# quanwei0/RAGEN

Hardware: AMD Instinct MI355X
Metric: env-steps/sec (whole node), Sokoban 6x6, 8192 envs x 5 turns (higher is better)
Workload: dtype u8

## Files before the change

ragen_amd/csrc/board_step.hpp:

```cpp
#pragma once
#include <stdint.h>
#if defined(__HIPCC__)
#include <hip/hip_runtime.h>
#endif

#include "ragen_amd.h"

#if defined(__HIP_DEVICE_COMPILE__)
#define RMI_BS_FN __device__ __forceinline__
#elif defined(__HIPCC__)
#define RMI_BS_FN __host__ __device__ __forceinline__
#else
#define RMI_BS_FN inline
#endif

namespace rmi {
namespace bs {

RMI_BS_FN uint32_t ubfe(uint32_t x, uint32_t off, uint32_t w) {
#if defined(__HIP_DEVICE_COMPILE__)
  return __builtin_amdgcn_ubfe(x, off, w);
#else
  off &= 31u;
  w &= 31u;
  return w ? (x >> off) & ((1u << w) - 1u) : 0u;
#endif
}
RMI_BS_FN uint32_t smask(uint32_t x, uint32_t off, uint32_t w) {
#if defined(__HIP_DEVICE_COMPILE__)
  return (uint32_t)__builtin_amdgcn_sbfe((int32_t)x, off, w);
#else
  off &= 31u;
  w &= 31u;
  return w ? (uint32_t)((int32_t)(x << (32u - off - w)) >> (32u - w)) : 0u;
#endif
}
template <class T>
RMI_BS_FN void opaque(T& x) {
#if defined(__HIP_DEVICE_COMPILE__)
  asm("" : "+v"(x));
#else
  (void)x;
#endif
}
RMI_BS_FN int32_t sbyte(uint32_t x, uint32_t off) {
#if defined(__HIP_DEVICE_COMPILE__)
  return __builtin_amdgcn_sbfe((int32_t)x, off, 8u);
#else
  return (int32_t)(int8_t)(uint8_t)(x >> off);
#endif
}
RMI_BS_FN uint32_t pick_bytes(uint32_t table, uint32_t sel) {
#if defined(__HIP_DEVICE_COMPILE__)
  return __builtin_amdgcn_perm(0u, table, sel);
#else
  uint32_t r = 0;
  for (int i = 0; i < 4; ++i) r |= ((table >> (8 * ((sel >> (8 * i)) & 3u))) & 0xFFu) << (8 * i);
  return r;
#endif
}
RMI_BS_FN int popc32(uint32_t x) { return __builtin_popcount(x); }
RMI_BS_FN int popc64(uint64_t x) { return __builtin_popcountll(x); }

template <class M>
struct Word;
template <>
struct Word<uint32_t> {
  static RMI_BS_FN uint32_t mask(uint32_t x, int j) { return smask(x, (uint32_t)j, 1u); }
  static RMI_BS_FN uint32_t at(int j) { return 1u << (j & 31); }
  static RMI_BS_FN uint32_t widen(uint32_t m) { return m; }
  static RMI_BS_FN int popc(uint32_t x) { return popc32(x); }
};
template <>
struct Word<uint64_t> {
  static RMI_BS_FN uint32_t mask(uint64_t x, int j) { return 0u - ((uint32_t)(x >> (j & 63)) & 1u); }
  static RMI_BS_FN uint64_t at(int j) { return 1ull << (j & 63); }
  static RMI_BS_FN uint64_t widen(uint32_t m) { return (uint64_t)(int64_t)(int32_t)m; }
  static RMI_BS_FN int popc(uint64_t x) { return popc64(x); }
};

RMI_BS_FN uint32_t valid_bytes(uint32_t x, uint32_t in_range) {
  return ((((x & 0x7F7F7F7Fu) + 0x7F7F7F7Fu) | x) & 0x80808080u) & in_range;
}

struct Slots4 {
  uint32_t V, P, D, S;
};
RMI_BS_FN Slots4 slots4(uint32_t x, uint32_t valid, uint32_t below, uint32_t left_b, uint32_t m_b, uint32_t dir_table) {
  Slots4 s;
  const uint32_t pc = (valid >> 7) * 0x01010101u + below;
  s.V = ((left_b | 0x80808080u) - pc) & valid;
  s.P = s.V & ~((x & 0x7F7F7F7Fu) + 0x7B7B7B7Bu);
  s.D = s.V & ~((pc ^ m_b) + 0x7F7F7F7Fu);
  s.S = pick_bytes(dir_table, x & 0x03030303u);
  return s;
}

struct BoardTurn {
  double acc;
  uint32_t info, taken, stop, succ, moved;
  int nes, bot;
};

template <class M, int K>
RMI_BS_FN BoardTurn board_turn_k(M wall, M target, M& box, int& jp, int W, uint64_t acts, int n_act, int left,
                                 int nes, int bot, int num_boxes, int max_steps) {
  const M box0 = box;
  const int jp0 = jp;
  const uint32_t dir_table = 0x01u | ((uint32_t)(-W) & 0xFFu) << 8 | ((uint32_t)W & 0xFFu) << 16 | 0xFF000000u;
  const uint64_t range = n_act >= 8 ? ~0ull : (1ull << (8 * n_act)) - 1;
  const uint32_t l8 = left <= 0 ? 0u : (left >= 8 ? 8u : (uint32_t)left);
  const int m = max_steps - nes;
  const uint32_t m8 = (m >= 1 && m <= 8) ? (uint32_t)m : 0x7Fu;
  const uint32_t left_b = l8 * 0x01010101u, m_b = m8 * 0x01010101u;
  const uint32_t xl = (uint32_t)acts, xh = (uint32_t)(acts >> 32);
  const uint32_t vl = valid_bytes(xl, (uint32_t)range);
  Slots4 q[2];
  q[0] = slots4(xl, vl, 0u, left_b, m_b, dir_table);
  if (K > 4) q[1] = slots4(xh, valid_bytes(xh, (uint32_t)(range >> 32)), (uint32_t)popc32(vl) * 0x01010101u, left_b, m_b, dir_table);
  uint32_t alive = 1u, taken = 0u, last_moved = 0u, z = 1u;
  int open_bot = num_boxes - bot;
  double acc = 0.0;
#pragma unroll
  for (int k = 0; k < K; ++k) {
    const Slots4& v = q[k >> 2];
    const uint32_t hb = 8u * (uint32_t)(k & 3) + 7u;
    const int s = sbyte(v.S, 8u * (uint32_t)(k & 3));
    const uint32_t go = smask(v.V, hb, alive), go_push = smask(v.P, hb, alive), go_done = smask(v.D, hb, alive);
    const int jn = jp + s, jb = jn + s;
    const M occ = wall | box;
    const uint32_t n_box = Word<M>::mask(box, jn), n_occ = Word<M>::mask(occ, jn), b_occ = Word<M>::mask(occ, jb);
    const uint32_t is_push = go_push & n_box & ~b_occ;
    const uint32_t moved = go & (is_push | ~n_occ);
    box ^= (Word<M>::at(jn) | Word<M>::at(jb)) & Word<M>::widen(is_push);
    jp = (int)((moved & (uint32_t)jn) | (~moved & (uint32_t)jp));
    const int n_open = Word<M>::popc(target & ~box);
    int sg = n_open - open_bot;
    sg = sg > 1 ? 1 : (sg < -1 ? -1 : sg);
    z = n_open < 1 ? (uint32_t)n_open : 1u;
    uint32_t fin = 1u - z;
    opaque(sg);
    opaque(fin);
    double rw = -0.1 - (double)sg;
    rw = __builtin_fma(10.0, (double)fin, rw);
    acc = __builtin_fma(-(double)(int32_t)go, rw, acc);
    open_bot = (int)((go & (uint32_t)n_open) | (~go & (uint32_t)open_bot));
    taken -= go;
    last_moved = (go & moved) | (~go & last_moved);
    alive &= ~(go_done | (go & fin));
  }
  BoardTurn t;
  t.acc = acc;
  t.taken = taken;
  t.stop = alive ^ 1u;
  t.succ = taken ? (z ^ 1u) : 0u;
  t.info = taken ? (RMI_INFO_PRESENT | RMI_INFO_VALID | (last_moved & 2u) | (t.succ << 3)) : 0u;
  t.moved = (box != box0) | (jp != jp0);
  t.nes = nes + (int)taken;
  t.bot = num_boxes - open_bot;
  return t;
}

}
}
```

ragen_amd/csrc/sokoban.hip:

```cpp
#include "common.hpp"
#include "board_step.hpp"
#include "parse_core.hpp"

#include <type_traits>

namespace rmi {
namespace {

constexpr int kWave = 64;
constexpr int kMaxCells = 64;

__device__ __forceinline__ uint32_t zero_bytes(uint32_t y) {
  return ~(((y & 0x7F7F7F7Fu) + 0x7F7F7F7Fu) | y) & 0x80808080u;
}
__device__ __forceinline__ uint32_t eq_bytes(uint32_t x, uint32_t v) { return zero_bytes(x ^ (v * 0x01010101u)); }

struct SokobanLdsEnv {
  uint8_t* st;
  const uint8_t* fx;
  int H, W, r, c;
  int num_env_steps, boxes_on_target, num_boxes, max_steps, n_open;
  uint8_t err;

  __device__ __forceinline__ int wrap(int row, int col, bool& ok) const {
    ok = row >= -H && row < H && col >= -W && col < W;
    const int rr = row < 0 ? row + H : row, cc = col < 0 ? col + W : col;
    return ok ? rr * W + cc : 0;
  }
  __device__ __forceinline__ static int open_of(int v, int f) { return (v == 2) | ((v == 5) & (f == 2)); }

  __device__ __forceinline__ bool step(int a, double& reward, bool& done, bool& eff, bool& success) {
    if (a < 1 || a > 8) return false;
    const int d = (a - 1) & 3;
    const int dr = d == 0 ? -1 : (d == 1 ? 1 : 0);
    const int dc = d == 2 ? -1 : (d == 3 ? 1 : 0);
    const int nr = r + dr, nc = c + dc, br = nr + dr, bc = nc + dc;
    bool ok_n, ok_b, ok_o;
    const int ni = wrap(nr, nc, ok_n), bi = wrap(br, bc, ok_b), oi = wrap(r, c, ok_o);
    const int vn = st[ni], vb = st[bi], vo = st[oi];
    const int fn = fx[ni], fb = fx[bi], fo = fx[oi];
    const bool push_act = a <= 4;
    const bool high = br >= H || bc >= W;
    const bool is_push = push_act && !high && (vn == 3 || vn == 4) && (vb == 1 || vb == 2);
    const bool try_move = !push_act || (!high && !is_push);
    const bool moved = is_push || (try_move && (vn == 1 || vn == 2));
    if ((push_act && !high && (!ok_n || !ok_b)) || (try_move && !ok_n) || (moved && !ok_o)) {
      err |= RMI_ERR_INDEX;
      return false;
    }
    num_env_steps += 1;
    const int vbn = fb == 2 ? 3 : 4;
    if (moved) {
      n_open += open_of(5, fn) - open_of(vn, fn) + open_of(fo, fo) - open_of(vo, fo);
      st[ni] = 5;
      st[oi] = (uint8_t)fo;
      r = nr;
      c = nc;
    }
    if (is_push) {
      n_open += open_of(vbn, fb) - open_of(vb, fb);
      st[bi] = (uint8_t)vbn;
    }
    const int cur = num_boxes - n_open;
    double rw = -0.1;
    rw += cur > boxes_on_target ? 1.0 : (cur < boxes_on_target ? -1.0 : 0.0);
    const bool all_on = n_open == 0;
    rw += all_on ? 10.0 : 0.0;
    boxes_on_target = cur;
    reward = rw;
    done = all_on || (max_steps == num_env_steps);
    success = boxes_on_target == num_boxes;
    eff = moved;
    return true;
  }
};

struct ExecList {
  uint64_t run;
  int cnt;
};
__device__ __forceinline__ ExecList exec_list(uint64_t acts, int n_act, int left) {
  ExecList x;
  x.run = 0;
  x.cnt = 0;
#pragma unroll
  for (int k = 0; k < kMaxK; ++k) {
    const uint32_t a = (uint32_t)(acts >> (8 * k)) & 0xFFu;
    const bool take = k < n_act && a != 0 && x.cnt < left;
    x.run |= take ? ((uint64_t)a << (8 * x.cnt)) : 0ull;
    x.cnt += take;
  }
  return x;
}

__device__ __forceinline__ void finish_turn(const TurnOut& o, bool turn_done, bool succ_last, int32_t& num_actions,
                                            uint8_t& flags, int32_t& n_turns, int max_actions) {
  num_actions += o.exec;
  n_turns += 1;
  if (turn_done) {
    flags |= RMI_FLAG_TERMINATED | RMI_FLAG_DONE;
    flags = succ_last ? (uint8_t)(flags & ~RMI_FLAG_TRUNCATED) : (uint8_t)(flags | RMI_FLAG_TRUNCATED);
  } else if (num_actions >= max_actions) {
    flags |= RMI_FLAG_TERMINATED | RMI_FLAG_TRUNCATED | RMI_FLAG_DONE;
  }
}

__device__ __forceinline__ double step_reward(int n_open, int num_boxes, int& boxes_on_target, bool& all_on) {
  const int cur = num_boxes - n_open;
  double rw = -0.1;
  rw += cur > boxes_on_target ? 1.0 : (cur < boxes_on_target ? -1.0 : 0.0);
  all_on = n_open == 0;
  rw += all_on ? 10.0 : 0.0;
  boxes_on_target = cur;
  return rw;
}


__device__ __forceinline__ uint32_t nonzero_bytes(uint32_t y) {
  return (((y & 0x7F7F7F7Fu) + 0x7F7F7F7Fu) | y) & 0x80808080u;
}
__device__ __forceinline__ uint32_t gt8_bytes(uint32_t y) {
  return (y | ((y & 0x7F7F7F7Fu) + 0x77777777u)) & 0x80808080u;
}
__device__ __forceinline__ uint32_t nib(uint32_t x) { return (x * 0x01020408u) >> 24; }
__device__ __forceinline__ uint32_t nib2(uint32_t x0, uint32_t x1) {
  return ((x0 | (x1 << 4)) * 0x00204081u) >> 21 & 0xFFu;
}
__device__ __forceinline__ uint32_t byte_mask(uint32_t x) { return (0x80808080u - x) ^ 0x80808080u; }

template <int LPE>
__device__ __forceinline__ uint32_t env_or(uint32_t x) {
  if (LPE >= 2) x |= (uint32_t)__builtin_amdgcn_mov_dpp((int)x, 0xB1, 0xF, 0xF, false);
  if (LPE >= 4) x |= (uint32_t)__builtin_amdgcn_mov_dpp((int)x, 0x4E, 0xF, 0xF, false);
  if (LPE >= 8) x |= (uint32_t)__builtin_amdgcn_mov_dpp((int)x, 0x141, 0xF, 0xF, false);
  if (LPE >= 16) x |= (uint32_t)__builtin_amdgcn_mov_dpp((int)x, 0x140, 0xF, 0xF, false);
  static_assert(LPE <= 16, "an env's lanes lie in one DPP row");
  return x;
}
template <int LPE>
__device__ __forceinline__ uint64_t env_or64(uint64_t x) {
  return ((uint64_t)env_or<LPE>((uint32_t)(x >> 32)) << 32) | env_or<LPE>((uint32_t)x);
}

template <int NWL, int LPE>
__device__ __forceinline__ bool decode_rows(const uint32_t (&xs)[NWL], const uint32_t (&xf)[NWL], int sub,
                                            int row_words, int p, uint64_t& wall, uint64_t& target, uint64_t& box) {
  constexpr uint32_t L = 0x01010101u;
  const int pw = p >> 2;
  const uint32_t pmask = 0xFFu << (8 * (p & 3)), p5 = 5u << (8 * (p & 3));
  uint32_t bad = 0;
  uint64_t wl = 0, tl = 0, bl = 0;
  uint32_t fw[NWL], ft[NWL], bx[NWL];
#pragma unroll
  for (int i = 0; i < NWL; ++i) {
// ... 564 lines not shown
        if (w < row_words) {
          ls[w] = xs[i];
          lf[w] = xf[i];
        }
      }
    }
    wave_sync();
    if (act && sub == 0) {
      int n_open = 0;
      for (int w = 0; w < row_words; ++w)
        n_open += __popc(eq_bytes(ls[w], 2u) | (eq_bytes(ls[w], 5u) & eq_bytes(lf[w], 2u)));
      SokobanLdsEnv e;
      e.st = reinterpret_cast<uint8_t*>(ls);
      e.fx = reinterpret_cast<const uint8_t*>(lf);
      e.H = H;
      e.W = W;
      e.r = r;
      e.c = c;
      e.num_env_steps = nes;
      e.boxes_on_target = bot;
      e.num_boxes = env.num_boxes;
      e.max_steps = env.max_steps;
      e.n_open = n_open;
      e.err = 0;
      const ExecList x = exec_list(acts, n_act, left);
      o = lds_turn(e, x, err, turn_done, succ_last);
      err |= e.err;
      r = e.r;
      c = e.c;
      nes = e.num_env_steps;
      bot = e.boxes_on_target;
      row_changed = o.stepped_any_state;
    }
    wave_sync();
    row_changed = env_or<LPE>(row_changed) != 0;
    if (act && row_changed) {
#pragma unroll
      for (int i = 0; i < NWL; ++i) {
        const int w = sub + LPE * i;
        if (w < row_words) xs[i] = ls[w];
      }
    }
  }
  RMI_STAMP(3);

  if (kFirst && live && !act && sub == 0) {
    elem<Ix>(env.player, 2 * b)[0] = (int8_t)r;
    elem<Ix>(env.player, 2 * b)[1] = (int8_t)c;
    *elem<Ix>(env.num_env_steps, b) = 0;
    *elem<Ix>(env.boxes_on_target, b) = 0;
    *elem<Ix>(ep.num_actions, b) = 0;
    *elem<Ix>(ep.flags, b) = 0;
    *elem<Ix>(ep.n_turns, b) = 0;
    *elem<Ix>(ep.penalty, b) = 0.0;
  }
  if (kFirst && live && sub == 0)
    for (int t = 0; t < ep.T; ++t)
      if (t != in.turn || !act) {
        *elem<Ix>(ep.turn_reward + (int64_t)t * B, b) = 0.0;
        *elem<Ix>(ep.turn_info + (int64_t)t * B, b) = 0;
        *elem<Ix>(ep.turn_exec + (int64_t)t * B, b) = 0;
      }
  if (act) {
    if (sub == 0) {
      finish_turn(o, turn_done, succ_last, num_actions, flags, n_turns, in.max_actions_per_traj);
      *elem<Ix>(ep.num_actions, b) = num_actions;
      *elem<Ix>(ep.flags, b) = flags;
      *elem<Ix>(ep.n_turns, b) = n_turns;
      *elem<Ix>(ep.penalty, b) = penalty;
      const int64_t tb = (int64_t)in.turn * B;
      *elem<Ix>(ep.turn_reward + tb, b) = o.acc;
      *elem<Ix>(ep.turn_info + tb, b) = o.info;
      *elem<Ix>(ep.turn_exec + tb, b) = o.exec;
      if (kFirst || o.stepped_any_state) {
        elem<Ix>(env.player, 2 * b)[0] = (int8_t)r;
        elem<Ix>(env.player, 2 * b)[1] = (int8_t)c;
        *elem<Ix>(env.num_env_steps, b) = nes;
        *elem<Ix>(env.boxes_on_target, b) = bot;
      }
      if (err_out && err) *elem<Ix>(err_out, b) |= err;
    }
    if (row_changed) store_row<NWL, LPE, HW != 0>(elem<Ix>(env.room_state, b * hw), xs, sub, row_words);
  }
  if (bmode != RMI_BOARDS_NONE && live) {
    const bool stepped_fast = fast && act;
    const bool write = bmode == RMI_BOARDS_BUILD || act || kFirst;
    const uint32_t tag = (stepped_fast || !act) ? (from_cache || room_ok ? 1u : 0u) : 0u;
    if (write) {
      const uint32_t cell = (uint32_t)(jp + W) & 0xFFu;
      *elem<Ix>(reinterpret_cast<Dw4*>(env.boards), b) = Dw4{(uint32_t)wall, (uint32_t)target, (uint32_t)box,
                                                   cell | (tag << 8) | ((uint32_t)nes & 0xFFu) << 16 |
                                                       ((uint32_t)bot & 0xFFu) << 24};
    }
  }
  RMI_STAMP(4);
  at_end(xs, xf, wall, target, box, (fast && act) ? jp : INT32_MIN);
  if (kFin) {
    if (act) rec.set(in.turn, o.acc, o.info);
    finalize_envs<LPE, Ix>(ep, fin, rec, b, live && sub == 0, flags, n_turns, num_actions, penalty, act ? in.turn : -1,
                       o.acc, o.info);
  }
}

template <int HW, class M, int LPE, bool kFin, bool kFirst = false, bool kLate = false, bool kObs = false,
          class Ix = int64_t>
__global__ __launch_bounds__(kWave * kSokWpb * (kObs ? kObsFan : 1)) void sokoban_step_turn_kernel(rmi_sokoban_t env, rmi_episode_t ep, rmi_turn_t in,
                                                                  int hw_rt, uint32_t w_magic, uint64_t border,
                                                                  uint8_t* __restrict__ err_out, rmi_finalize_t fin,
                                                                  const uint8_t* __restrict__ init_state = nullptr,
                                                                  const int8_t* __restrict__ init_player = nullptr,
                                                                  ObsOut obs = ObsOut{}) {
  static_assert(!kObs || (HW == 36 && LPE == 1 && !kLate), "the fused render: 36-cell rooms, one lane per env");
  constexpr int NW = HW ? HW / 4 : kMaxWords;
  constexpr int kEnvs = kWave / LPE;
  __shared__ uint32_t lds_state[kSokWpb * kEnvs * NW];
  __shared__ uint32_t lds_fixed[kSokWpb * kEnvs * NW];
  using ObsL = ObsLds<kObs ? HW : 36, M>;
  __shared__ typename std::conditional<kObs, ObsL, char>::type lds_obs;
  const int B = ep.B;
  const int lane = threadIdx.x & (kWave - 1), wave = threadIdx.x / kWave;
  const int sub = lane % LPE, slot = lane / LPE;
  const bool turn_wave = !kObs || wave < kSokWpb;
  const int64_t b = turn_wave ? ((int64_t)blockIdx.x * kSokWpb + wave) * kEnvs + slot : (int64_t)B;
  const int row_words = (HW ? HW : hw_rt) >> 2;
  auto at_end = [&](const auto& xs, const auto& xf, M wall, M target, M box, int jp) {
        if constexpr (kObs) {
          const int H = env.H, W = env.W;
          if (turn_wave) {
            const int e = wave * kWave + lane;
#pragma unroll
            for (int i = 0; i < NW; ++i) {
              lds_obs.xs[e][i] = xs[i];
              lds_obs.xf[e][i] = xf[i];
            }
            lds_obs.wall[e] = wall;
            lds_obs.target[e] = target;
            lds_obs.box[e] = box;
            lds_obs.jp[e] = jp;
          }
          if (threadIdx.x < 18) lds_obs.gb[threadIdx.x] = threadIdx.x < 16 ? obs.gb[threadIdx.x] : (threadIdx.x == 16 ? '?' : '\n');
          __syncthreads();
#ifndef RMI_OBS_SKIP_RENDER
          render_group<HW, M>(obs, lds_obs, B, H, W);
#endif
        }
      };
  constexpr bool kBoards = HW == 36 && LPE == 1 && !kLate && !kObs && sizeof(M) == 4;
  static_assert(sizeof(Ix) == 8 || kBoards, "32-bit env offsets: the SK layout only (launched below kOff32MaxB envs)");
  turn_env<HW, M, LPE, kFin, kFirst, kLate, kBoards, Ix>(env, ep, in, hw_rt, w_magic, border, err_out, fin, init_state,
                                                         init_player, b, sub, lds_state + (wave * kEnvs + slot) * row_words,
                                                         lds_fixed + (wave * kEnvs + slot) * row_words, at_end);
}

__global__ __launch_bounds__(kBlock) void sokoban_reset_kernel(rmi_sokoban_t env, rmi_episode_t ep, int hw,
                                                               const uint8_t* __restrict__ init_state,
                                                               const int8_t* __restrict__ init_player) {
  const int64_t i = (int64_t)blockIdx.x * kBlock + threadIdx.x;
  const int64_t B = ep.B;
  const int64_t nwords = (B * hw) >> 2;
  if (i < nwords) reinterpret_cast<uint32_t*>(env.room_state)[i] = reinterpret_cast<const uint32_t*>(init_state)[i];
  if (i < B) {
    env.player[2 * i] = init_player[2 * i];
    env.player[2 * i + 1] = init_player[2 * i + 1];
    env.num_env_steps[i] = 0;
    env.boxes_on_target[i] = 0;
    ep.num_actions[i] = 0;
    ep.flags[i] = 0;
    ep.n_turns[i] = 0;
    ep.penalty[i] = 0.0;
    for (int t = 0; t < ep.T; ++t) {
      ep.turn_reward[t * B + i] = 0.0;
      ep.turn_info[t * B + i] = 0;
      ep.turn_exec[t * B + i] = 0;
    }
  }
}

__global__ __launch_bounds__(kBlock) void sokoban_load_rooms_kernel(rmi_sokoban_t env, rmi_episode_t ep, int hw,
                                                                    const uint8_t* __restrict__ rooms, int n_rooms,
                                                                    const int32_t* __restrict__ room_of,
                                                                    uint8_t* __restrict__ init_state,
                                                                    int8_t* __restrict__ init_player,
                                                                    uint8_t* __restrict__ err) {
  const int64_t t = (int64_t)blockIdx.x * kBlock + threadIdx.x;
  const int64_t B = ep.B;
  const int64_t pitch = 2 * hw + 2;
  if (t < B * hw) {
    const int64_t i = t / hw;
    const int k = (int)(t - i * hw);
    const int r = room_of ? room_of[i] : (int)i;
    const bool bad = r < 0 || r >= n_rooms;
    const uint8_t f = bad ? 0 : rooms[(int64_t)r * pitch + k], v = bad ? 0 : rooms[(int64_t)r * pitch + hw + k];
    const_cast<uint8_t*>(env.room_fixed)[t] = f;
    env.room_state[t] = v;
    init_state[t] = v;
  }
  if (t < B) {
    const int64_t i = t;
    const int r = room_of ? room_of[i] : (int)i;
    const bool bad = r < 0 || r >= n_rooms;
    if (err) err[i] = bad ? RMI_ERR_INDEX : 0;
    const uint8_t* src = rooms + (int64_t)(bad ? 0 : r) * pitch + 2 * hw;
    const int8_t p0 = bad ? 0 : (int8_t)src[0], p1 = bad ? 0 : (int8_t)src[1];
    init_player[2 * i] = p0;
    init_player[2 * i + 1] = p1;
    env.player[2 * i] = p0;
    env.player[2 * i + 1] = p1;
    env.num_env_steps[i] = 0;
    env.boxes_on_target[i] = 0;
    ep.num_actions[i] = 0;
    ep.flags[i] = 0;
    ep.n_turns[i] = 0;
    ep.penalty[i] = 0.0;
    for (int u = 0; u < ep.T; ++u) {
      ep.turn_reward[u * B + i] = 0.0;
      ep.turn_info[u * B + i] = 0;
      ep.turn_exec[u * B + i] = 0;
    }
  }
}


constexpr int kTokEnvs = 16;
#ifdef RMI_TOK_STAMPS
__device__ unsigned long long* g_tok_stamps;
#define TST_DECL unsigned long long tst_[8] = {0}; tst_[0] = __builtin_amdgcn_s_memrealtime(); tst_[1] = __builtin_amdgcn_s_memtime()
#define TST(i) (tst_[i] = __builtin_amdgcn_s_memtime())
#define TST_FLUSH(w)                                                                              \
  do {                                                                                            \
    tst_[7] = __builtin_amdgcn_s_memrealtime();                                                   \
    if ((threadIdx.x & 63) == 0 && g_tok_stamps)                                                  \
      for (int s_ = 0; s_ < 8; ++s_) g_tok_stamps[((int64_t)blockIdx.x * kTokEnvs + (w)) * 8 + s_] = tst_[s_]; \
  } while (0)
#else
#define TST_DECL do {} while (0)
#define TST(i) do {} while (0)
#define TST_FLUSH(w) do {} while (0)
#endif
constexpr int kTokRowWords = 48;
struct TokRec {
  uint32_t xs[9], xf[9];
  uint32_t wall, target, box;
  int jp;
};
__host__ __device__ constexpr size_t tok_static_lds() {
  return 2 * kTokEnvs * 9 * 4 + kTokEnvs * sizeof(TokRec) + kTokEnvs * kTokRowWords * 4 + 18 * 4;
}

template <bool kFin, bool kFirst>
__global__ __launch_bounds__(kWave* kTokEnvs) __attribute__((amdgpu_waves_per_eu(8))) void sokoban_token_turn_kernel(
    DetokArgs d, ParseArgs a, rmi_sokoban_t env, rmi_episode_t ep, rmi_turn_t in, uint32_t w_magic, uint64_t border,
    uint8_t* __restrict__ err_out, rmi_finalize_t fin, const uint8_t* __restrict__ init_state,
    const int8_t* __restrict__ init_player, ObsOut obs, const uint8_t* __restrict__ has_t, uint8_t* __restrict__ has) {
  extern __shared__ uint64_t lds_q[];
  __shared__ uint32_t lds_state[kTokEnvs * 9], lds_fixed[kTokEnvs * 9];
  __shared__ TokRec rec[kTokEnvs];
  __shared__ uint32_t blk[kTokEnvs][kTokRowWords];
  __shared__ uint32_t gb[18];
  __shared__ struct {
    uint8_t* out;
    int32_t* len;
    uint64_t glen;
    int stride, H, W, B;
  } rp;
  const int wv = __builtin_amdgcn_readfirstlane(threadIdx.x >> 6), lane = threadIdx.x & 63;
  const int64_t b0 = (int64_t)blockIdx.x * kTokEnvs, b = b0 + wv;
  TST_DECL;
  if (threadIdx.x < 18) gb[threadIdx.x] = threadIdx.x < 16 ? obs.gb[threadIdx.x] : (threadIdx.x == 16 ? '?' : '\n');
  if (threadIdx.x == 64) {
    rp.out = obs.out;
    rp.len = obs.len;
    rp.glen = obs.glen;
    rp.stride = obs.stride;
    rp.H = env.H;
    rp.W = env.W;
    rp.B = ep.B;
  }

  if (b < a.B) {
    uint8_t* lds = reinterpret_cast<uint8_t*>(lds_q) + wv * parse_lds(a.stride);
    const int cap = list_cap(a.stride);
    uint8_t* T = lds + 4;
    uint8_t* Wb = lds + row_bytes(a.stride) + 4;
    uint16_t* EL = reinterpret_cast<uint16_t*>(lds + 2 * row_bytes(a.stride));
    uint16_t* ES = EL + cap;
    uint8_t* EI = reinterpret_cast<uint8_t*>(ES + cap);
    const Names nm = load_names(a.cfg, (a.sel && a.sel[b]) ? 1 : 0);
#ifdef RMI_PARSE_STAMPS
    unsigned long long pst_[10], dst_[6];
#endif
    uint8_t derr;
    const int n = detok_row(d, T + kPre, Wb + kPre, b, lane DSTAMP_ARG, &derr);
    if (has && lane == 0) {
      has[b] = ((!has_t || has_t[b]) && derr == 0) ? 1 : 0;
      err_out[b] = 0;
    }
    parse_row(a, T, Wb, EL, ES, EI, b, n, 0, nm, lane PSTAMP_ARG);
  }
  TST(2);
  __syncthreads();
  TST(3);

  constexpr int kLpeT = 16;
  constexpr int kTurnWaves = kTokEnvs * kLpeT / kWave;
#ifndef RMI_TOK_NO_TURN
  if (wv < kTurnWaves) {
    const int t = wv * kWave + lane, e = t / kLpeT, sub = t % kLpeT;
    const int64_t be = b0 + e;
    turn_env<36, uint32_t, kLpeT, false, kFirst, false, false, int64_t, false>(
        env, ep, in, 36, w_magic, border, err_out, fin, init_state, init_player, be, sub, lds_state + e * 9, lds_fixed + e * 9,
        [&](const auto& xs, const auto& xf, uint32_t wall, uint32_t target, uint32_t box, int jp) {
#pragma unroll
          for (int i = 0; i < (9 + kLpeT - 1) / kLpeT; ++i) {
            const int w = sub + kLpeT * i;
            if (w < 9) {
              rec[e].xs[w] = xs[i];
              rec[e].xf[w] = xf[i];
            }
          }
          if (sub == 0) {
            rec[e].wall = wall;
            rec[e].target = target;
            rec[e].box = box;
            rec[e].jp = jp;
          }
        });
  }
#endif
  TST(4);
  __syncthreads();
  TST(5);
  if constexpr (kFin) {
    if (wv == 0) {
      const int64_t be = b0 + (lane & (kTokEnvs - 1)), bc = be < ep.B ? be : (int64_t)ep.B - 1;
      FinRecord fr;
      fr.load(ep, bc);
      finalize_envs<1>(ep, fin, fr, be, lane < kTokEnvs && be < ep.B, ep.flags[bc], ep.n_turns[bc],
                       ep.num_actions[bc], ep.penalty[bc], -1, 0.0, 0);
    }
  }
#ifdef RMI_TOK_NO_RENDER
  return;
#endif

  if (b >= rp.B) {
    TST_FLUSH(wv);
    return;
  }
  const int H = rp.H, W = rp.W, T = H * (W + 1) - 1;
  const TokRec& R = rec[wv];
  const int r = lane / (W + 1), c = lane - r * (W + 1);
  uint32_t cd = 0x100u;
  if (lane < T) {
    if (c == W) {
      cd = 0xFFu;
    } else {
      const int i = r * W + c;
      const uint32_t s_ = (R.xs[i >> 2] >> (8 * (i & 3))) & 0xFFu, f_ = (R.xf[i >> 2] >> (8 * (i & 3))) & 0xFFu;
      int v = (s_ == 5u && f_ == 2u) ? 6 : (int)s_;
      if (R.jp != INT32_MIN) {
        const int qb = i - W, qq = qb >= 0 ? qb : 0;
        const uint32_t wl = qb >= 0 ? (R.wall >> qq) & 1u : 1u;
        const int tg = (int)((R.target >> qq) & 1u), bx = (int)((R.box >> qq) & 1u);
        v = wl ? 0 : (qb == R.jp ? 5 + tg : (bx ? 4 - tg : 1 + tg));
      }
      cd = (uint32_t)(v > 0xFE ? 0xFE : v);
    }
  }
  const uint32_t g = gb[cd < 16u ? cd : (cd == 0xFFu ? 17u : 16u)];
  const int len = cd == 0x100u ? 0 : (cd < 16u ? (int)((rp.glen >> (4 * cd)) & 15u) : 1);
  const int incl = wave_inclusive_scan(len);
  const int off = incl - len, total = __builtin_amdgcn_readlane(incl, 63), nw = (total + 3) >> 2;
  uint32_t* row = blk[wv];
  if (lane < nw) row[lane] = 0u;
  wave_sync();
  uint8_t* rb = reinterpret_cast<uint8_t*>(row);
#pragma unroll
  for (int q = 0; q < 4; ++q)
    if (q < len) rb[off + q] = (uint8_t)(g >> (8 * q));
  wave_sync();
  if (lane < nw) reinterpret_cast<uint32_t*>(rp.out + b * (int64_t)rp.stride)[lane] = row[lane];
  if (lane == 0) rp.len[b] = total;
  TST(6);
  TST_FLUSH(wv);
}

}
}

#ifndef RMI_SOK_LATE_MIN
#define RMI_SOK_LATE_MIN (1 << 17)
#endif
namespace rmi {
namespace {
inline uint32_t w_magic_of(int W) { return (65536u + (uint32_t)W - 1u) / (uint32_t)W; }

template <bool kFin, bool kFirst = false>
int sokoban_step_turn_launch(const rmi_sokoban_t* env, const rmi_episode_t* ep, const rmi_turn_t* in, uint8_t* err,
                             const rmi_finalize_t& fin, hipStream_t s, const uint8_t* init_state = nullptr,
                             const int8_t* init_player = nullptr) {
  const int hw = env->H * env->W;
  const unsigned grid = (unsigned)((ep->B + kWave * kSokWpb - 1) / (kWave * kSokWpb));
  const int H = env->H, W = env->W;
  uint64_t border = 0;
  for (int r = 0; r < H; ++r)
    for (int c = 0; c < W; ++c)
      if (r == 0 || c == 0 || r == H - 1 || c == W - 1) border |= 1ull << (r * W + c);
  const bool w32 = (H - 1) * W <= 32;
  const uint32_t w_magic = w_magic_of(W);
  const bool spread = spread_lanes(ep->B);
  const bool late = !kFirst && !spread && ep->B >= RMI_SOK_LATE_MIN;
  if (env->boards && (hw != 36 || !w32 || spread || ep->B >= RMI_SOK_LATE_MIN ||
                      (env->boards_mode != RMI_BOARDS_BUILD && env->boards_mode != RMI_BOARDS_USE) ||
                      ((reinterpret_cast<uintptr_t>(env->boards) | reinterpret_cast<uintptr_t>(env->init_boards)) & 15u)))
    return RMI_EUNSUP;
#define RMI_LAUNCH(HW_, M_)                                                                                   \
  do {                                                                                                        \
    if (spread)                                                                                               \
      hipLaunchKernelGGL((sokoban_step_turn_kernel<HW_, M_, kSpreadLpe, kFin, kFirst>),                       \
                         dim3((unsigned)((ep->B + kWave * kSokWpb / kSpreadLpe - 1) /                          \
                                         (kWave * kSokWpb / kSpreadLpe))),                                   \
                         dim3(kWave * kSokWpb), 0, s, *env, *ep, *in, hw, w_magic, border, err, fin, init_state, \
                         init_player);                                                                        \
    else if (late) {                                                                                          \
      if constexpr (!kFirst)                                                                                  \
        hipLaunchKernelGGL((sokoban_step_turn_kernel<HW_, M_, 1, kFin, false, true>), dim3(grid),            \
                           dim3(kWave * kSokWpb), 0, s, *env, *ep, *in, hw, w_magic, border, err, fin, init_state, \
                           init_player);                                                                      \
    } else {                                                                                                  \
      if constexpr (HW_ == 36 && sizeof(M_) == 4) {                                                           \
        if (ep->B < kOff32MaxB) {                                                                             \
          hipLaunchKernelGGL((sokoban_step_turn_kernel<HW_, M_, 1, kFin, kFirst, false, false, uint32_t>),    \
                             dim3(grid), dim3(kWave * kSokWpb), 0, s, *env, *ep, *in, hw, w_magic, border, err, fin, \
                             init_state, init_player);                                                        \
          break;                                                                                              \
        }                                                                                                     \
      }                                                                                                       \
      hipLaunchKernelGGL((sokoban_step_turn_kernel<HW_, M_, 1, kFin, kFirst>), dim3(grid), dim3(kWave * kSokWpb), \
                         0, s, *env, *ep, *in, hw, w_magic, border, err, fin, init_state, init_player);        \
    }                                                                                                         \
  } while (0)
  if (hw == 36 && w32)
    RMI_LAUNCH(36, uint32_t);
  else if (hw == 36)
    RMI_LAUNCH(36, uint64_t);
  else if (hw == 64)
    RMI_LAUNCH(64, uint64_t);
  else if (w32)
    RMI_LAUNCH(0, uint32_t);
  else
    RMI_LAUNCH(0, uint64_t);
#undef RMI_LAUNCH
  return launch_status();
}

template <bool kFin, bool kFirst>
int sokoban_step_turn_obs_launch(const rmi_sokoban_t* env, const rmi_episode_t* ep, const rmi_turn_t* in, uint8_t* err,
                                 const rmi_finalize_t& fin, hipStream_t s, const uint8_t* init_state,
                                 const int8_t* init_player, const ObsOut& obs) {
  const int hw = env->H * env->W;
  const int H = env->H, W = env->W;
  if (spread_lanes(ep->B) || hw != 36 || obs.stride > obs_pitch_max(hw)) return RMI_EUNSUP;
  uint64_t border = 0;
  for (int r = 0; r < H; ++r)
    for (int c = 0; c < W; ++c)
      if (r == 0 || c == 0 || r == H - 1 || c == W - 1) border |= 1ull << (r * W + c);
  const bool w32 = (H - 1) * W <= 32;
  const uint32_t w_magic = w_magic_of(W);
  const dim3 grid((unsigned)((ep->B + kWave * kSokWpb - 1) / (kWave * kSokWpb))), block(kWave * kSokWpb * kObsFan);
  if (w32)
    hipLaunchKernelGGL((sokoban_step_turn_kernel<36, uint32_t, 1, kFin, kFirst, false, true>), grid, block, 0, s, *env,
                       *ep, *in, hw, w_magic, border, err, fin, init_state, init_player, obs);
  else
    hipLaunchKernelGGL((sokoban_step_turn_kernel<36, uint64_t, 1, kFin, kFirst, false, true>), grid, block, 0, s, *env,
                       *ep, *in, hw, w_magic, border, err, fin, init_state, init_player, obs);
  return launch_status();
}

int sokoban_check(const rmi_sokoban_t* env) {
  if (!env) return RMI_EINVAL;
  const int hw = env->H * env->W;
  if (env->H <= 0 || env->W <= 0 || hw > kMaxCells) return RMI_EUNSUP;
  if (!env->room_fixed || !env->room_state || !env->player || !env->num_env_steps || !env->boxes_on_target)
    return RMI_EINVAL;
  if (hw % 4 != 0 ||
      ((reinterpret_cast<uintptr_t>(env->room_state) | reinterpret_cast<uintptr_t>(env->room_fixed)) & 3u))
    return RMI_EUNSUP;
  return RMI_OK;
}
}
}

#ifdef RMI_TOK_STAMPS
RMI_API int rmi_tok_set_stamps(unsigned long long* buf) {
  return hipMemcpyToSymbol(HIP_SYMBOL(rmi::g_tok_stamps), &buf, sizeof(buf)) == hipSuccess ? 0 : -2;
}
#endif
#ifdef RMI_STAMPS
RMI_API int rmi_sokoban_set_stamps(unsigned long long* buf) {
  return hipMemcpyToSymbol(HIP_SYMBOL(rmi::g_stamps), &buf, sizeof(buf)) == hipSuccess ? 0 : -2;
}
#endif

namespace rmi {
namespace {
constexpr int kSkip = 1;
int validate_turn(const rmi_sokoban_t* env, const rmi_episode_t* ep, const rmi_turn_t* in, const rmi_finalize_t* fin,
                  const uint8_t* init_state, const int8_t* init_player, rmi_finalize_t& f, bool boards_ok = false) {
  if (!env || (init_state && !ep)) return RMI_EINVAL;
  if (env->boards && !boards_ok) return RMI_EUNSUP;
  if (env->H <= 0 || env->W <= 0 || env->H * env->W > kMaxCells) return RMI_EUNSUP;
  const int rc = check_turn_args(ep, in);
  if (rc != RMI_OK) return rc > 0 ? kSkip : rc;
  const int ec = sokoban_check(env);
  if (ec != RMI_OK) return ec;
  f = rmi_finalize_t{};
  if (fin) {
    if (fin->method < 0 || fin->method > 3 || fin->group_size < 1) return RMI_EINVAL;
    const int per_wave = spread_lanes(ep->B) ? kWave / kSpreadLpe : kWave;
    if (per_wave % fin->group_size != 0 || ep->B % fin->group_size != 0) return RMI_EUNSUP;
    f = *fin;
    if (f.group_size == 1) f.method = RMI_NORM_IDENTITY;
  }
  if (init_state) {
    if (!init_player) return RMI_EINVAL;
    if (reinterpret_cast<uintptr_t>(init_state) & 3u) return RMI_EUNSUP;
  }
  return RMI_OK;
}
}
}

RMI_API int rmi_sokoban_step_turn(const rmi_sokoban_t* env, const rmi_episode_t* ep, const rmi_turn_t* in,
                                  uint8_t* err, rmi_stream_t stream) {
  using namespace rmi;
  rmi_finalize_t f;
  const int rc = validate_turn(env, ep, in, nullptr, nullptr, nullptr, f, true);
  if (rc != RMI_OK) return rc == kSkip ? RMI_OK : rc;
  return sokoban_step_turn_launch<false>(env, ep, in, err, f, as_stream(stream));
}

RMI_API int rmi_sokoban_step_turn_finalize(const rmi_sokoban_t* env, const rmi_episode_t* ep, const rmi_turn_t* in,
                                           uint8_t* err, const rmi_finalize_t* fin, rmi_stream_t stream) {
  using namespace rmi;
  if (!fin) return RMI_EINVAL;
  rmi_finalize_t f;
  const int rc = validate_turn(env, ep, in, fin, nullptr, nullptr, f, true);
  if (rc != RMI_OK) return rc == kSkip ? RMI_OK : rc;
  return sokoban_step_turn_launch<true>(env, ep, in, err, f, as_stream(stream));
}

RMI_API int rmi_sokoban_step_turn_first(const rmi_sokoban_t* env, const rmi_episode_t* ep, const rmi_turn_t* in,
                                        const uint8_t* init_state, const int8_t* init_player, uint8_t* err,
                                        rmi_stream_t stream) {
  using namespace rmi;
  if (!init_state || !init_player) return RMI_EINVAL;
  rmi_finalize_t f;
  const int rc = validate_turn(env, ep, in, nullptr, init_state, init_player, f, true);
  if (rc != RMI_OK) return rc == kSkip ? RMI_OK : rc;
  return sokoban_step_turn_launch<false, true>(env, ep, in, err, f, as_stream(stream), init_state, init_player);
}

namespace rmi {
namespace {
int obs_out(const rmi_sokoban_t* env, const rmi_render_t* obs, ObsOut& o) {
  if (!obs || !env || env->H <= 0 || env->W <= 0) return RMI_EINVAL;
  for (int k = 0; k < 16; ++k)
    if (obs->glyph_len[k] > 4) return RMI_EINVAL;
// ... 135 lines not shown
```

Measured before the change: 2.920 billion.

## Add lean cached-board turn kernel for 6x6 Sokoban with incremental room writes

Adds a specialized per-K kernel for 6x6 boards in boards-USE mode. It reads the cached bitboard entry directly, loads the action bytes as aligned dwords combined with alignbyte, and runs the bitboard turn. Only the cells that changed (player and boxes) are written back to room_state instead of the full row. Waves whose inputs are untagged or invalid fall back to the general turn_env path, which adds code size and template instances and raises some risk of divergence in flag and reward semantics.

```diff
diff --git a/ragen_amd/csrc/board_step.hpp b/ragen_amd/csrc/board_step.hpp
--- a/ragen_amd/csrc/board_step.hpp
+++ b/ragen_amd/csrc/board_step.hpp
@@ -102,22 +102,36 @@
   int nes, bot;
 };
 
+struct ValidSlots {
+  uint32_t lo, hi;
+};
+template <int K>
+RMI_BS_FN ValidSlots valid_slots(uint32_t xl, uint32_t xh, int n_act) {
+  ValidSlots v;
+  const uint32_t rl = n_act >= 4 ? ~0u : (1u << (8 * n_act)) - 1u;
+  v.lo = valid_bytes(xl, rl);
+  v.hi = 0u;
+  if (K > 4) {
+    const int nh = n_act - 4;
+    const uint32_t rh = nh >= 4 ? ~0u : (nh <= 0 ? 0u : (1u << (8 * nh)) - 1u);
+    v.hi = valid_bytes(xh, rh);
+  }
+  return v;
+}
+
 template <class M, int K>
-RMI_BS_FN BoardTurn board_turn_k(M wall, M target, M& box, int& jp, int W, uint64_t acts, int n_act, int left,
-                                 int nes, int bot, int num_boxes, int max_steps) {
+RMI_BS_FN BoardTurn board_turn_kv(M wall, M target, M& box, int& jp, int W, uint32_t xl, uint32_t xh, uint32_t vl,
+                                  uint32_t vh, int left, int nes, int bot, int num_boxes, int max_steps) {
   const M box0 = box;
   const int jp0 = jp;
   const uint32_t dir_table = 0x01u | ((uint32_t)(-W) & 0xFFu) << 8 | ((uint32_t)W & 0xFFu) << 16 | 0xFF000000u;
-  const uint64_t range = n_act >= 8 ? ~0ull : (1ull << (8 * n_act)) - 1;
   const uint32_t l8 = left <= 0 ? 0u : (left >= 8 ? 8u : (uint32_t)left);
   const int m = max_steps - nes;
   const uint32_t m8 = (m >= 1 && m <= 8) ? (uint32_t)m : 0x7Fu;
   const uint32_t left_b = l8 * 0x01010101u, m_b = m8 * 0x01010101u;
-  const uint32_t xl = (uint32_t)acts, xh = (uint32_t)(acts >> 32);
-  const uint32_t vl = valid_bytes(xl, (uint32_t)range);
   Slots4 q[2];
   q[0] = slots4(xl, vl, 0u, left_b, m_b, dir_table);
-  if (K > 4) q[1] = slots4(xh, valid_bytes(xh, (uint32_t)(range >> 32)), (uint32_t)popc32(vl) * 0x01010101u, left_b, m_b, dir_table);
+  if (K > 4) q[1] = slots4(xh, vh, (uint32_t)popc32(vl) * 0x01010101u, left_b, m_b, dir_table);
   uint32_t alive = 1u, taken = 0u, last_moved = 0u, z = 1u;
   int open_bot = num_boxes - bot;
   double acc = 0.0;
@@ -161,5 +175,15 @@
   return t;
 }
 
+template <class M, int K>
+RMI_BS_FN BoardTurn board_turn_k(M wall, M target, M& box, int& jp, int W, uint64_t acts, int n_act, int left,
+                                 int nes, int bot, int num_boxes, int max_steps) {
+  const uint64_t range = n_act >= 8 ? ~0ull : (1ull << (8 * n_act)) - 1;
+  const uint32_t xl = (uint32_t)acts, xh = (uint32_t)(acts >> 32);
+  const uint32_t vl = valid_bytes(xl, (uint32_t)range);
+  const uint32_t vh = K > 4 ? valid_bytes(xh, (uint32_t)(range >> 32)) : 0u;
+  return board_turn_kv<M, K>(wall, target, box, jp, W, xl, xh, vl, vh, left, nes, bot, num_boxes, max_steps);
+}
+
 }
 }
diff --git a/ragen_amd/csrc/lean_turn.hpp b/ragen_amd/csrc/lean_turn.hpp
--- /dev/null
+++ b/ragen_amd/csrc/lean_turn.hpp
@@ -0,0 +1,48 @@
+#pragma once
+#include <stdint.h>
+
+#include "board_step.hpp"
+
+namespace rmi {
+namespace lean {
+
+RMI_BS_FN uint32_t align_bytes(uint32_t hi, uint32_t lo, uint32_t sh) {
+#if defined(__HIP_DEVICE_COMPILE__)
+  return __builtin_amdgcn_alignbyte(hi, lo, sh);
+#else
+  return (uint32_t)(((((uint64_t)hi) << 32) | lo) >> (8u * (sh & 3u)));
+#endif
+}
+
+template <int K>
+struct ActionLoads {
+  static_assert(K >= 1 && K <= 8, "1..8 action slots");
+  static constexpr int kDwords = K <= 1 ? 1 : (K <= 5 ? 2 : 3);
+};
+
+struct ActionAddr {
+  uint32_t o0, o1, o2, sh;
+};
+template <int K>
+RMI_BS_FN ActionAddr action_addr(uint32_t b, uint32_t mis) {
+  const uint32_t o = b * (uint32_t)K + mis;
+  ActionAddr a;
+  a.sh = o & 3u;
+  const uint32_t last = (a.sh + (uint32_t)K - 1u) >> 2;
+  a.o0 = o & ~3u;
+  a.o1 = a.o0 + (last >= 1u ? 4u : 0u);
+  a.o2 = a.o0 + 4u * (last >= 2u ? 2u : last);
+  return a;
+}
+
+template <int K>
+RMI_BS_FN void action_bytes(uint32_t d0, uint32_t d1, uint32_t d2, uint32_t sh, uint32_t& lo, uint32_t& hi) {
+  constexpr int kN = ActionLoads<K>::kDwords;
+  lo = kN == 1 ? d0 >> (8u * (sh & 3u)) : align_bytes(d1, d0, sh);
+  hi = K > 4 ? align_bytes(kN == 3 ? d2 : d1, d1, sh) : 0u;
+  if (K < 4) lo &= (1u << (8 * (K & 3))) - 1u;
+  if (K > 4 && K < 8) hi &= (1u << (8 * (K & 3))) - 1u;
+}
+
+}
+}
diff --git a/ragen_amd/csrc/sokoban.hip b/ragen_amd/csrc/sokoban.hip
--- a/ragen_amd/csrc/sokoban.hip
+++ b/ragen_amd/csrc/sokoban.hip
@@ -1,5 +1,6 @@
 #include "common.hpp"
 #include "board_step.hpp"
+#include "lean_turn.hpp"
 #include "parse_core.hpp"
 
 #include <type_traits>
@@ -870,6 +871,196 @@
                                                          lds_fixed + (wave * kEnvs + slot) * row_words, at_end);
 }
 
+constexpr uint64_t border_cells(int H, int W) {
+  uint64_t m = 0;
+  for (int r = 0; r < H; ++r)
+    for (int c = 0; c < W; ++c)
+      if (r == 0 || c == 0 || r == H - 1 || c == W - 1) m |= 1ull << (r * W + c);
+  return m;
+}
+
+__device__ __forceinline__ uint8_t cell_byte(uint32_t target, uint32_t box, uint32_t pl, int j) {
+  const uint32_t sel = bs::ubfe(target, (uint32_t)j, 1u) | bs::ubfe(box, (uint32_t)j, 1u) << 1 |
+                       bs::ubfe(pl, (uint32_t)j, 1u) << 2;
+  return (uint8_t)__builtin_amdgcn_perm(0x05050505u, 0x03040201u, sel);
+}
+
+template <int K, bool kFirst, bool kFin, bool kHasInput>
+__global__ __launch_bounds__(kWave * kSokWpb) void sokoban_cached_turn_kernel(
+    rmi_sokoban_t env_arg, rmi_episode_t ep_arg, rmi_turn_t in_arg, uint8_t* __restrict__ err_out, rmi_finalize_t fin,
+    const uint8_t* __restrict__ init_state, const int8_t* __restrict__ init_player, double* rec_reward,
+    uint8_t* rec_info, uint8_t* rec_exec) {
+  static_assert(!(kFirst && kFin), "a first turn that is also the last is launched as the general kernel");
+  using Ix = uint32_t;
+  using M = uint32_t;
+  constexpr int W = 6, HW = 36, NW = HW / 4;
+  constexpr uint32_t kWMagic = (65536u + W - 1u) / W;
+  __shared__ uint32_t lds_state[kSokWpb * kWave * NW];
+  __shared__ uint32_t lds_fixed[kSokWpb * kWave * NW];
+  RMI_STAMP_DECL;
+  RMI_STAMP(0);
+  rmi_sokoban_t env = env_arg;
+  rmi_episode_t ep = ep_arg;
+  rmi_turn_t in = in_arg;
+  const uint8_t* reset_rows = init_state;
+  if (kFirst || kFin) args_pin(ep.T, ep.turn_reward, ep.turn_info, in.turn);
+  if (kFirst) args_pin(ep.turn_exec, reset_rows, env.init_boards);
+  if (kHasInput) args_pin(in.has_input);
+  args_pin(ep.B, env.num_boxes, env.max_steps, env.room_state, env.player, env.num_env_steps, env.boxes_on_target,
+           env.boards, ep.num_actions, ep.flags, ep.n_turns, ep.penalty, in.actions, in.n_actions,
+           in.max_actions_per_traj, in.format_penalty, rec_reward, rec_info, rec_exec);
+
+  const uint32_t B = (uint32_t)ep.B;
+  const uint32_t b = blockIdx.x * (uint32_t)(kWave * kSokWpb) + threadIdx.x;
+  const bool live = b < B;
+  const uint32_t bc = live ? b : B - 1u;
+
+  const Dw4 ent = *elem<Ix>(reinterpret_cast<const Dw4*>(kFirst ? env.init_boards : env.boards), bc);
+  uint32_t xs[NW];
+  if (kFirst) load_row<NW, 1, true>(elem<Ix>(reset_rows, bc * HW), xs, 0, NW);
+  uint8_t has_in = 0;
+  if (kHasInput) has_in = *elem<Ix>(in.has_input, bc);
+  uint8_t flags = 0;
+  int32_t num_actions = 0, n_turns = 0;
+  double penalty = 0.0;
+  if (!kFirst) {
+    flags = *elem<Ix>(ep.flags, bc);
+    num_actions = *elem<Ix>(ep.num_actions, bc);
+    n_turns = *elem<Ix>(ep.n_turns, bc);
+    penalty = *elem<Ix>(ep.penalty, bc);
+  }
+  int n_act = *elem<Ix>(in.n_actions, bc);
+  uint32_t al, ah;
+  {
+    constexpr int kN = lean::ActionLoads<K>::kDwords;
+    const uint32_t mis = (uint32_t)(reinterpret_cast<uintptr_t>(in.actions) & 3u);
+    const char* abase = (const char*)in.actions - mis;
+    const lean::ActionAddr ad = lean::action_addr<K>(bc, mis);
+    const uint32_t d0 = *(const uint32_t*)(abase + ad.o0);
+    uint32_t d1 = 0, d2 = 0;
+    if (kN >= 2) d1 = *(const uint32_t*)(abase + ad.o1);
+    if (kN >= 3) d2 = *(const uint32_t*)(abase + ad.o2);
+    lean::action_bytes<K>(d0, d1, d2, ad.sh, al, ah);
+  }
+  FinRecord rec;
+  if (kFin) rec.load<Ix>(ep, bc);
+  if (!live) flags = RMI_FLAG_DONE;
+  const bool act = live && (kHasInput ? has_in != 0 : !(flags & RMI_FLAG_DONE));
+
+  if (n_act > K) n_act = K;
+  const bs::ValidSlots vs = bs::valid_slots<K>(al, ah, n_act);
+  const bool acts_ok = ((gt8_bytes(al) & vs.lo) | (K > 4 ? gt8_bytes(ah) & vs.hi : 0u)) == 0;
+  const bool tagged = (ent.w >> 8 & 0xFFu) == 1u;
+  const int lean_ok = kFirst ? (!live) | (tagged & (acts_ok | !act)) : (!act) | (tagged & acts_ok);
+  if (kFirst) {
+#pragma unroll
+    for (int i = 0; i < NW; ++i) asm volatile("" : "+v"(xs[i]));
+  } else {
+    asm volatile("" : "+v"(num_actions), "+v"(n_turns), "+v"(penalty));
+  }
+  if (__builtin_expect(!__all(lean_ok), 0)) {
+    constexpr uint64_t kBorder = border_cells(W, W);
+    const int lane = threadIdx.x & (kWave - 1), wave = threadIdx.x / kWave;
+    turn_env<HW, M, 1, kFin, kFirst, false, true, Ix, false>(
+        env_arg, ep_arg, in_arg, HW, kWMagic, kBorder, err_out, fin, init_state, init_player, (int64_t)b, 0,
+        lds_state + (wave * kWave + lane) * NW, lds_fixed + (wave * kWave + lane) * NW,
+        [](const auto&, const auto&, M, M, M, int) {});
+    return;
+  }
+  RMI_STAMP_WAIT(1);
+  if (kFirst && live) store_row<NW, 1, true>(elem<Ix>(env.room_state, b * HW), xs, 0, NW);
+
+  M wall = ent.x, target = ent.y, box = ent.z;
+  int jp = (int)(ent.w & 0xFFu) - W;
+  int nes = (int)(ent.w >> 16 & 0xFFu), bot = (int)(int8_t)(ent.w >> 24);
+  RMI_STAMP(2);
+
+  double acc = 0.0;
+  uint8_t info = 0;
+  uint32_t taken = 0;
+  if (act) {
+    flags &= (uint8_t)~RMI_FLAG_DONE;
+    const int nv = __popc(vs.lo) + (K > 4 ? __popc(vs.hi) : 0);
+    if (nv != n_act || nv == 0) penalty += in.format_penalty;
+    const int left = in.max_actions_per_traj - num_actions;
+    const M box0 = box;
+    const int jp0 = jp;
+    const BoardTurn t = bs::board_turn_kv<M, K>(wall, target, box, jp, W, al, ah, vs.lo, vs.hi, left, nes, bot,
+                                                env.num_boxes, env.max_steps);
+    nes = t.nes;
+    bot = t.bot;
+    acc = t.acc;
+    info = (uint8_t)t.info;
+    taken = t.taken;
+    if (t.moved) {
+      const M pl = (M)1 << jp;
+      M m = (box0 ^ box) | ((M)1 << jp0) | pl;
+      const uint32_t win = b * HW + W;
+      int jj[4];
+      jj[0] = __builtin_ctz(m);
+      m &= m - 1;
+#pragma unroll
+      for (int k = 1; k < 4; ++k) {
+        jj[k] = m ? __builtin_ctz(m) : jj[0];
+        m &= m - 1;
+      }
+#pragma unroll
+      for (int k = 0; k < 4; ++k) *elem<Ix>(env.room_state, win + jj[k]) = cell_byte(target, box, pl, jj[k]);
+      while (m) {
+        const int j = __builtin_ctz(m);
+        m &= m - 1;
+        *elem<Ix>(env.room_state, win + j) = cell_byte(target, box, pl, j);
+      }
+    }
+    num_actions += (int32_t)taken;
+    n_turns += 1;
+    if (t.stop) {
+      flags |= RMI_FLAG_TERMINATED | RMI_FLAG_DONE;
+      flags = t.succ ? (uint8_t)(flags & ~RMI_FLAG_TRUNCATED) : (uint8_t)(flags | RMI_FLAG_TRUNCATED);
+    } else if (num_actions >= in.max_actions_per_traj) {
+      flags |= RMI_FLAG_TERMINATED | RMI_FLAG_TRUNCATED | RMI_FLAG_DONE;
+    }
+    *elem<Ix>(ep.num_actions, b) = num_actions;
+    *elem<Ix>(ep.flags, b) = flags;
+    *elem<Ix>(ep.n_turns, b) = n_turns;
+    *elem<Ix>(ep.penalty, b) = penalty;
+    *elem<Ix>(rec_reward, b) = acc;
+    *elem<Ix>(rec_info, b) = info;
+    *elem<Ix>(rec_exec, b) = (uint8_t)taken;
+  }
+  RMI_STAMP(3);
+  if (kFirst ? live : (act && taken != 0)) {
+    const uint32_t p = (uint32_t)(jp + W);
+    const uint32_t r = (p * kWMagic) >> 16, c = p - r * W;
+    *elem<Ix>(reinterpret_cast<uint16_t*>(env.player), b) = (uint16_t)(r | c << 8);
+    *elem<Ix>(env.num_env_steps, b) = nes;
+    *elem<Ix>(env.boxes_on_target, b) = bot;
+  }
+  if (kFirst && live) {
+    if (!act) {
+      *elem<Ix>(ep.num_actions, b) = 0;
+      *elem<Ix>(ep.flags, b) = 0;
+      *elem<Ix>(ep.n_turns, b) = 0;
+      *elem<Ix>(ep.penalty, b) = 0.0;
+    }
+    for (int t = 0; t < ep.T; ++t)
+      if (t != in.turn || !act) {
+        *elem<Ix>(ep.turn_reward + (int64_t)t * B, b) = 0.0;
+        *elem<Ix>(ep.turn_info + (int64_t)t * B, b) = 0;
+        *elem<Ix>(ep.turn_exec + (int64_t)t * B, b) = 0;
+      }
+  }
+  if (kFirst ? live : act)
+    *elem<Ix>(reinterpret_cast<Dw4*>(env.boards), b) =
+        Dw4{wall, target, box, ((uint32_t)(jp + W) & 0xFFu) | 1u << 8 | ((uint32_t)nes & 0xFFu) << 16 |
+                                   ((uint32_t)bot & 0xFFu) << 24};
+  RMI_STAMP(4);
+  if (kFin) {
+    if (act) rec.set(in.turn, acc, info);
+    finalize_envs<1, Ix>(ep, fin, rec, b, live, flags, n_turns, num_actions, penalty, act ? in.turn : -1, acc, info);
+  }
+}
+
 __global__ __launch_bounds__(kBlock) void sokoban_reset_kernel(rmi_sokoban_t env, rmi_episode_t ep, int hw,
                                                                const uint8_t* __restrict__ init_state,
                                                                const int8_t* __restrict__ init_player) {
@@ -1113,6 +1304,30 @@
 namespace {
 inline uint32_t w_magic_of(int W) { return (65536u + (uint32_t)W - 1u) / (uint32_t)W; }
 
+template <bool kFin, bool kFirst, bool kHasInput>
+void cached_turn_launch(const rmi_sokoban_t* env, const rmi_episode_t* ep, const rmi_turn_t* in, uint8_t* err,
+                        const rmi_finalize_t& fin, hipStream_t s, const uint8_t* init_state, const int8_t* init_player,
+                        unsigned grid) {
+  const int64_t tb = (int64_t)in->turn * ep->B;
+#define RMI_CACHED_K(k_)                                                                                          \
+  case k_:                                                                                                        \
+    hipLaunchKernelGGL((sokoban_cached_turn_kernel<k_, kFirst, kFin, kHasInput>), dim3(grid), dim3(kWave * kSokWpb), \
+                       0, s, *env, *ep, *in, err, fin, init_state, init_player, ep->turn_reward + tb,              \
+                       ep->turn_info + tb, ep->turn_exec + tb);                                                    \
+    break;
+  switch (in->K) {
+    RMI_CACHED_K(1)
+    RMI_CACHED_K(2)
+    RMI_CACHED_K(3)
+    RMI_CACHED_K(4)
+    RMI_CACHED_K(5)
+    RMI_CACHED_K(6)
+    RMI_CACHED_K(7)
+    RMI_CACHED_K(8)
+  }
+#undef RMI_CACHED_K
+}
+
 template <bool kFin, bool kFirst = false>
 int sokoban_step_turn_launch(const rmi_sokoban_t* env, const rmi_episode_t* ep, const rmi_turn_t* in, uint8_t* err,
                              const rmi_finalize_t& fin, hipStream_t s, const uint8_t* init_state = nullptr,
@@ -1132,6 +1347,14 @@
                       (env->boards_mode != RMI_BOARDS_BUILD && env->boards_mode != RMI_BOARDS_USE) ||
                       ((reinterpret_cast<uintptr_t>(env->boards) | reinterpret_cast<uintptr_t>(env->init_boards)) & 15u)))
     return RMI_EUNSUP;
+  if (H == 6 && W == 6 && !spread && ep->B < RMI_SOK_LATE_MIN && ep->B < kOff32MaxB && env->boards &&
+      env->boards_mode == RMI_BOARDS_USE && (!kFirst || env->init_boards) && in->K >= 1) {
+    if (in->has_input)
+      cached_turn_launch<kFin, kFirst, true>(env, ep, in, err, fin, s, init_state, init_player, grid);
+    else
+      cached_turn_launch<kFin, kFirst, false>(env, ep, in, err, fin, s, init_state, init_player, grid);
+    return launch_status();
+  }
 #define RMI_LAUNCH(HW_, M_)                                                                                   \
   do {                                                                                                        \
     if (spread)                                                                                               \
```

Measured after the change: 3.328 billion (median of 6 runs). 1.14x the previous value.
